# leotimus/recommender-tensorflow

Hardware: AMD Instinct MI355X
Metric: examples/sec DeepFM batch=65536 (full train step) (higher is better)
Workload: dtype f32 (MLP GEMM operands: fp16 hi+lo split, 3 products, fp32 accumulate)

## Files before the change

include/mi355x_rec.h:

```cpp
#ifndef MI355X_REC_H
#define MI355X_REC_H

#include <stddef.h>
#include <stdint.h>

#ifdef __cplusplus
extern "C" {
#endif

typedef void* mi_stream_t;

enum mi_status {
  MI_OK = 0,
  MI_ERR_INVALID = -1,
  MI_ERR_UNSUPPORTED = -2,
  MI_ERR_LAUNCH = -3,
  MI_ERR_WORKSPACE = -4
};

int32_t mi_abi_version(void);
const char* mi_last_error(void);
const char* mi_build_info(void);

typedef struct mi_step_state {
// ... 90 lines not shown
  MI_OPT_ADAGRAD = 1,
  MI_OPT_FTRL = 2,
  MI_OPT_RMSPROP = 3,
  MI_OPT_SGD = 4
};

typedef struct mi_opt_hparams {
  int32_t kind;
  float lr;
  float beta1, beta2, epsilon;
  float lr_t;
  float decay, momentum;
  float lr_power, l1, l2;
} mi_opt_hparams;

int32_t mi_axpy(float* y, const float* x, int64_t n, float alpha, mi_stream_t stream);

int32_t mi_dense_apply(float* param, float* slot0, float* slot1, const float* grad, int64_t n,
                       const mi_opt_hparams* hp, mi_stream_t stream);

int32_t mi_sparse_apply(float* table, float* t_slot0, float* t_slot1, float* lin_w, float* l_slot0,
                        float* l_slot1, int32_t* last_step, const int32_t* uniq_rows,
                        const int32_t* seg_start, const int32_t* sorted_entry,
                        const int32_t* num_uniq, int64_t n_max, const float* d_rows,
                        const float* d_lin, int32_t E, int32_t step, const mi_opt_hparams* hp,
                        int32_t lin_stride, int64_t table_stride, int64_t grad_stride, mi_stream_t stream);

int32_t mi_sparse_apply_fused(float* table, float* t_slot0, float* t_slot1, float* lin_w, float* l_slot0,
                              float* l_slot1, int32_t* last_step, const int32_t* uniq_rows,
                              const int32_t* seg_start, const int32_t* sorted_entry, const int32_t* num_uniq,
                              int64_t n_max, const float* d_concat, int64_t ld_dconcat, const float* sumv,
                              const float* d_logit_fm, const float* d_logit_lin, int32_t F, int32_t E,
                              int32_t step, const mi_opt_hparams* hp, int32_t lin_stride, int64_t table_stride, mi_stream_t stream);

enum mi_catchup_flags { MI_CATCHUP_DEFER_SLOTS = 1, MI_CATCHUP_BOUNDED = 2, MI_CATCHUP_KEEP_STAMPS = 4, MI_CATCHUP_LOCAL_ORDER = 8 };
int32_t mi_catchup_local_chunk_rows(void);
int32_t mi_catchup_bounded_runs(float beta1, float beta2, float epsilon);
int32_t mi_catchup_local_plan(int64_t n_max, int64_t num_uniq, int64_t* plan);
int32_t mi_catchup_gap_keys(const int32_t* uniq_rows, const int32_t* num_uniq, const int32_t* last_step, int64_t n_max,
                            int32_t step_to, int32_t* keys, int32_t lin_stride, mi_stream_t stream);

int32_t mi_catchup_rows_by_gap(const int32_t* uniq_rows, const int32_t* num_uniq, const int32_t* last_step, int64_t n_max,
                               int32_t step_to, int32_t lin_stride, int32_t* rows_out, void* workspace,
                               size_t workspace_bytes, mi_stream_t stream);


int32_t mi_selftest_sqrt(uint32_t first_bits, int64_t count, uint64_t* mismatches, mi_stream_t stream);

int32_t mi_selftest_div(float d, uint32_t first_bits, int64_t count, uint64_t* out, mi_stream_t stream);

int32_t mi_sparse_catchup(float* table, float* t_m, float* t_v, float* lin_w, float* l_m, float* l_v,
                          int32_t* last_step, const int32_t* uniq_rows, const int32_t* num_uniq,
                          int64_t n_max, int32_t E, int32_t step_to, const float* lr_table,
                          float beta1, float beta2, float epsilon, int32_t flags, int32_t lin_stride,
                          int64_t table_stride, mi_stream_t stream);


int32_t mi_set_gemm_mode(int32_t mode);
int32_t mi_get_gemm_mode(void);

#define MI_AMAX_SLOTS 64
typedef struct mi_gemm_amax {
  const float* a;
  const float* b;
  float* out;
} mi_gemm_amax_t;
// ... 238 lines not shown
```

recommender-tensorflow_amd/csrc/optim.hip:

```cpp
#include "common.h"
#include "optim_rules.h"
#include <algorithm>

namespace {

constexpr int kBlock = 256;

__global__ __launch_bounds__(kBlock) void dense_apply_k(float* __restrict__ w, float* __restrict__ s0,
                                                        float* __restrict__ s1,
                                                        const float* __restrict__ g, int64_t n,
                                                        Hp h, const mi_step_state_t* __restrict__ st) {
  if (st) h.lr_t = st->lr_t;
  const int64_t stride = static_cast<int64_t>(gridDim.x) * kBlock;
  for (int64_t i = static_cast<int64_t>(blockIdx.x) * kBlock + threadIdx.x; i < n; i += stride) {
    float wv = w[i], a = s0 ? s0[i] : 0.f, b = s1 ? s1[i] : 0.f;
    dense_rule(h, wv, a, b, g[i]);
    w[i] = wv;
    if (s0) s0[i] = a;
    if (s1) s1[i] = b;
  }
}

typedef float f32x4_t __attribute__((ext_vector_type(4)));
__device__ __forceinline__ float4 ld4_nt(const float* p) {
  const f32x4_t v = __builtin_nontemporal_load(reinterpret_cast<const f32x4_t*>(p));
  return make_float4(v[0], v[1], v[2], v[3]);
}
__device__ __forceinline__ void st4_nt(float* p, float4 v) {
  const f32x4_t x = {v.x, v.y, v.z, v.w};
  __builtin_nontemporal_store(x, reinterpret_cast<f32x4_t*>(p));
}

struct FusedGrad {
  const float* d_concat; int64_t ldd; const float* sumv; const float* dlf; const float* dll; int F;
  int64_t b0;
};

constexpr int kLongSeg = 48;
constexpr int kRun = 1;

struct ApplyArgs {
  float* table; float* t0; float* t1;
  float* lin_w; float* l0; float* l1;
  int32_t* last_step;
  const int32_t* uniq_rows; const int32_t* seg_start; const int32_t* sorted_entry; const int32_t* num_uniq;
  const float* d_rows; const float* d_lin;
  int E, step;
  float* out_rows; float* out_lin; int u_begin, u_count;
  int ls;
  const mi_step_state_t* st;
  int64_t ts;
  int64_t gs, gls, os, ols;
};

template <bool FUSED>
__device__ __forceinline__ void seg_accumulate(const ApplyArgs& a, const FusedGrad& fg, int k_beg, int k_end, int l,
                                               bool lane_on, const float4& w, float4& g, float& gl) {
  const int E = a.E;
  for (int k = k_beg; k < k_end; ++k) {
    const int64_t e = a.sorted_entry[k];
    if constexpr (FUSED) {
      const int64_t bg = e / fg.F;
      const int f = static_cast<int>(e - bg * fg.F);
      const int64_t b = bg - fg.b0;
      if (a.table && lane_on) {
        float4 v = make_float4(0.f, 0.f, 0.f, 0.f);
        if (fg.d_concat) v = ld4(fg.d_concat + b * fg.ldd + static_cast<int64_t>(f) * E + 4 * l);
        if (fg.dlf) {
          const float gf = fg.dlf[b];
          if (fg.sumv) {
            const float4 sv = ld4(fg.sumv + b * E + 4 * l);
            v.x += gf * (sv.x - w.x); v.y += gf * (sv.y - w.y);
            v.z += gf * (sv.z - w.z); v.w += gf * (sv.w - w.w);
          } else {
            v.x -= gf * w.x; v.y -= gf * w.y; v.z -= gf * w.z; v.w -= gf * w.w;
          }
        }
        g.x += v.x; g.y += v.y; g.z += v.z; g.w += v.w;
      }
      if (a.lin_w && l == 0) gl += fg.dll[b];
    } else {
      if (a.table && lane_on) {
        const float4 v = ld4(a.d_rows + e * a.gs + 4 * l);
        g.x += v.x; g.y += v.y; g.z += v.z; g.w += v.w;
      }
      if (a.lin_w && l == 0) gl += a.d_lin[e * a.gls];
// ... 38 lines not shown
    sparse_rule(h, w.z, s0.z, s1.z, g.z);
    sparse_rule(h, w.w, s0.w, s1.w, g.w);
    st4(a.table + o, w);
    if (a.t0) st4_nt(a.t0 + o, s0);
    if (a.t1) st4_nt(a.t1 + o, s1);
  }
  if (l == 0) {
    if (a.lin_w) {
      const int64_t o = r * a.ls;
      float lw = q.lw, s0 = q.ls0, s1 = q.ls1;
      for (int j = 0; j < missed; ++j) { s0 = s0 * h.beta1; s1 = s1 * h.beta2; }
      sparse_rule(h, lw, s0, s1, gl);
      a.lin_w[o] = lw;
      if (a.l0) a.l0[o] = s0;
      if (a.l1) a.l1[o] = s1;
    }
    if (a.last_step) a.last_step[r * a.ls] = a.step;
  }
}

__device__ __forceinline__ void store_row(const ApplyArgs& a, int64_t u, int l, bool lane_on, const float4& g, float gl) {
  if (a.out_rows && lane_on) st4(a.out_rows + u * a.os + 4 * l, g);
  if (a.out_lin && l == 0) a.out_lin[u * a.ols] = gl;
}

template <int LPR, bool FUSED, bool STORE = false>
__global__ __launch_bounds__(kBlock) void sparse_apply_k(ApplyArgs a, Hp h, const FusedGrad fg) {
  if (a.st) { a.step = a.st->step; h.lr_t = a.st->lr_t; }
  int64_t u = (static_cast<int64_t>(blockIdx.x) * kBlock + threadIdx.x) / LPR;
  const int l = threadIdx.x & (LPR - 1);
  if (u >= (STORE ? a.u_count : *a.num_uniq)) return;
  if (STORE) u += a.u_begin;
  const int s_beg = a.seg_start[u], s_end = a.seg_start[u + 1];
  if (s_end - s_beg > kLongSeg) return;
  const int64_t r = STORE ? u : static_cast<int64_t>(a.uniq_rows[u]);
  const bool lane_on = 4 * l < a.E;
  float4 g = make_float4(0.f, 0.f, 0.f, 0.f);
  float gl = 0.f;
  float4 w = make_float4(0.f, 0.f, 0.f, 0.f);
  if (a.table && lane_on) w = ld4(a.table + r * a.ts + 4 * l);
  RowState q;
  if constexpr (!STORE) q = load_row_state(a, h, r, l, lane_on);
  seg_accumulate<FUSED>(a, fg, s_beg, s_end, l, lane_on, w, g, gl);
  if constexpr (STORE) store_row(a, u, l, lane_on, g, gl);
  else apply_row(a, h, r, l, lane_on, w, g, gl, q);
}

template <int LPR, bool FUSED, bool STORE = false>
__global__ __launch_bounds__(kBlock) void sparse_apply_long_k(ApplyArgs a, Hp h, const FusedGrad fg) {
  if (a.st) { a.step = a.st->step; h.lr_t = a.st->lr_t; }
  constexpr int G = kBlock / LPR;
  __shared__ int list[kBlock];
  __shared__ int n_list;
  __shared__ float4 part[kBlock];
  __shared__ float part_l[G];
  const int U = STORE ? a.u_count : *a.num_uniq;
  const int ub = STORE ? a.u_begin : 0;
  const int t = threadIdx.x, l = t & (LPR - 1), grp = t / LPR;
  const bool lane_on = 4 * l < a.E;
  const int64_t per_round = static_cast<int64_t>(kBlock) * gridDim.x;
  {
    int any = 0;
    for (int64_t base = 0; base < U; base += per_round) {
      const int64_t u = base + (static_cast<int64_t>(t / kRun) * gridDim.x + blockIdx.x) * kRun + t % kRun;
      if (u < U) any |= (a.seg_start[ub + u + 1] - a.seg_start[ub + u] > kLongSeg) ? 1 : 0;
    }
    if (!__syncthreads_or(any)) return;
  }
  for (int64_t base = 0; base < U; base += per_round) {
    if (t == 0) n_list = 0;
    __syncthreads();
    const int64_t u = base + (static_cast<int64_t>(t / kRun) * gridDim.x + blockIdx.x) * kRun + t % kRun;
    if (u < U && a.seg_start[ub + u + 1] - a.seg_start[ub + u] > kLongSeg) list[atomicAdd(&n_list, 1)] = static_cast<int>(ub + u);
    __syncthreads();
    const int n = n_list;
    for (int j = 0; j < n; ++j) {
      const int uu = list[j];
      const int64_t r = STORE ? static_cast<int64_t>(uu) : static_cast<int64_t>(a.uniq_rows[uu]);
      const int s_beg = a.seg_start[uu], s_end = a.seg_start[uu + 1];
      const int per = (s_end - s_beg + G - 1) / G;
      const int k0 = min(s_end, s_beg + grp * per), k1 = min(s_end, k0 + per);
      float4 g = make_float4(0.f, 0.f, 0.f, 0.f);
      float gl = 0.f;
      float4 w = make_float4(0.f, 0.f, 0.f, 0.f);
      if (a.table && lane_on) w = ld4(a.table + r * a.ts + 4 * l);
      seg_accumulate<FUSED>(a, fg, k0, k1, l, lane_on, w, g, gl);
      part[t] = g;
      if (l == 0) part_l[grp] = gl;
      __syncthreads();
      if (grp == 0) {
        g = part[l];
        gl = part_l[0];
#pragma unroll 4
        for (int q = 1; q < G; ++q) {
          const float4 v = part[q * LPR + l];
          g.x += v.x; g.y += v.y; g.z += v.z; g.w += v.w;
          gl += part_l[q];
        }
        if constexpr (STORE) store_row(a, uu, l, lane_on, g, gl);
        else apply_row(a, h, r, l, lane_on, w, g, gl, load_row_state(a, h, r, l, lane_on));
      }
      __syncthreads();
    }
  }
}

__device__ __forceinline__ float sqrt_rn_fixup(float x) {
  float s = __builtin_amdgcn_sqrtf(x);
  const float sm = __uint_as_float(__float_as_uint(s) - 1u), sp = __uint_as_float(__float_as_uint(s) + 1u);
  const float rm = fmaf(-sm, s, x), rp = fmaf(-sp, s, x);
  s = (rm <= 0.f) ? sm : s;
  s = (rp > 0.f) ? sp : s;
  return s;
}
__device__ __forceinline__ float sqrt_rn_inrange(float x) {
  const float r = __builtin_amdgcn_rsqf(x);
  float s = x * r, h = 0.5f * r;
  const float e = fmaf(-h, s, 0.5f);
  h = fmaf(h, e, h);
  s = fmaf(s, e, s);
  const float d = fmaf(-s, s, x);
  return fmaf(d, h, s);
}
__device__ __forceinline__ float div_rn_inrange(float n, float d) {
  float r = __builtin_amdgcn_rcpf(d);
  const float e = fmaf(-d, r, 1.0f);
  r = fmaf(e, r, r);
  float q = n * r;
  const float e2 = fmaf(-d, q, n);
  q = fmaf(e2, r, q);
  const float e3 = fmaf(-d, q, n);
  return fmaf(e3, r, q);
}
__device__ __forceinline__ bool catchup_in_range(float m, float v) {
  const float am = fabsf(m);
  return (am == 0.f || (am >= 0x1p-50f && am <= 0x1p60f)) && v >= 0x1p-93f && v <= 0x1p20f;
}
// ... 454 lines not shown

#define MI_DISPATCH_LPR(lpr, CALL)                  \
  switch (lpr) {                                    \
    case 1: { constexpr int L = 1; CALL; } break;   \
    case 2: { constexpr int L = 2; CALL; } break;   \
    case 4: { constexpr int L = 4; CALL; } break;   \
    case 8: { constexpr int L = 8; CALL; } break;   \
    case 16: { constexpr int L = 16; CALL; } break; \
    case 32: { constexpr int L = 32; CALL; } break; \
    default: { constexpr int L = 64; CALL; } break; \
  }

static int32_t check_hp(const char* who, const mi_opt_hparams* hp) {
  if (!hp || hp->kind < MI_OPT_ADAM || hp->kind > MI_OPT_SGD) {
    mi::set_error("%s: bad optimizer kind", who);
    return MI_ERR_INVALID;
  }
  if (hp->kind == MI_OPT_FTRL && hp->lr_power != -0.5f) {
    mi::set_error("%s: Ftrl learning_rate_power %f unsupported (TF default -0.5 only)", who, hp->lr_power);
    return MI_ERR_UNSUPPORTED;
  }
  return MI_OK;
}

__global__ __launch_bounds__(kBlock) void axpy_k(float* __restrict__ y, const float* __restrict__ x, int64_t n, float alpha) {
  const int64_t i = static_cast<int64_t>(blockIdx.x) * kBlock + threadIdx.x;
  if (i < n) y[i] = y[i] + alpha * x[i];
}

unsigned long_grid(int64_t n_max) {
  return static_cast<unsigned>(std::min<int64_t>(1024, mi::ceil_div(n_max, kBlock)));
}

__global__ void step_advance_k(mi_step_state_t* __restrict__ st, const float* __restrict__ lr_table) {
  const int s = st->step + 1;
  st->step = s;
  st->lr_t = lr_table ? lr_table[s] : 0.f;
  st->seed_term = static_cast<uint64_t>(s) * 1000003ull;
}

extern "C" {

int32_t mi_step_advance(mi_step_state_t* device_state, const float* lr_table, mi_stream_t stream) {
  MI_REQUIRE(device_state, "step_advance: null state");
  step_advance_k<<<dim3(1), dim3(1), 0, mi::as_stream(stream)>>>(device_state, lr_table);
  MI_CHECK_LAUNCH("step_advance");
  return MI_OK;
}

int32_t mi_axpy(float* y, const float* x, int64_t n, float alpha, mi_stream_t stream) {
  MI_REQUIRE(n >= 0 && (n == 0 || (x && y)), "axpy: n=%lld", (long long)n);
  if (n == 0) return MI_OK;
  axpy_k<<<dim3((unsigned)mi::ceil_div(n, kBlock)), dim3(kBlock), 0, mi::as_stream(stream)>>>(y, x, n, alpha);
  MI_CHECK_LAUNCH("axpy");
  return MI_OK;
}


int32_t mi_dense_apply(float* param, float* slot0, float* slot1, const float* grad, int64_t n,
                       const mi_opt_hparams* hp, mi_stream_t stream) {
  if (int32_t rc = check_hp("dense_apply", hp)) return rc;
  MI_REQUIRE(n >= 0, "dense_apply: n=%lld", (long long)n);
  if (n == 0) return MI_OK;
  MI_REQUIRE(param && grad, "dense_apply: null buffer");
  MI_REQUIRE(hp->kind == MI_OPT_SGD || slot0, "dense_apply: optimizer needs slot0");
  MI_REQUIRE((hp->kind != MI_OPT_ADAM && hp->kind != MI_OPT_FTRL && hp->kind != MI_OPT_RMSPROP) || slot1,
             "dense_apply: optimizer needs slot1");
  int64_t nb = mi::ceil_div(n, kBlock);
  if (nb > 4096) nb = 4096;
  dense_apply_k<<<dim3((unsigned)nb), dim3(kBlock), 0, mi::as_stream(stream)>>>(param, slot0, slot1, grad, n, make_hp(hp), mi::step_state());
  MI_CHECK_LAUNCH("dense_apply");
  return MI_OK;
}

int32_t mi_sparse_apply(float* table, float* t_slot0, float* t_slot1, float* lin_w, float* l_slot0,
                        float* l_slot1, int32_t* last_step, const int32_t* uniq_rows,
                        const int32_t* seg_start, const int32_t* sorted_entry,
                        const int32_t* num_uniq, int64_t n_max, const float* d_rows,
                        const float* d_lin, int32_t E, int32_t step, const mi_opt_hparams* hp,
                        int32_t lin_stride, int64_t table_stride, int64_t grad_stride, mi_stream_t stream) {
  if (int32_t rc = check_hp("sparse_apply", hp)) return rc;
  MI_REQUIRE(grad_stride == 0 || (grad_stride >= (table ? E : 1) && (!table || (grad_stride & 3) == 0)),
             "sparse_apply: grad_stride=%lld (0 = d_rows E apart and d_lin 1 apart, else one record per entry)", (long long)grad_stride);
  if (!table) table_stride = 0;
  MI_REQUIRE(table_stride == 0 || (table_stride >= E && (table_stride & 3) == 0), "%s: table_stride=%lld (0 = E, else >= E and a multiple of 4)", "sparse_apply", (long long)table_stride);
  const int64_t ts = table_stride ? table_stride : E;

  MI_REQUIRE(lin_stride >= 1, "sparse_apply: lin_stride=%d", lin_stride);
  MI_REQUIRE(n_max >= 0, "sparse_apply: n_max=%lld", (long long)n_max);
  if (n_max == 0) return MI_OK;
  MI_REQUIRE(table || lin_w, "sparse_apply: nothing to update");
  MI_REQUIRE(uniq_rows && seg_start && sorted_entry && num_uniq, "sparse_apply: null index buffer");
  MI_REQUIRE(!table || (d_rows && E >= 4 && E <= 256 && (E & 3) == 0 && mi::aligned16(table) && mi::aligned16(d_rows)),
             "sparse_apply: table needs d_rows, E multiple of 4 in [4,256], 16-byte alignment");
  MI_REQUIRE(!lin_w || d_lin, "sparse_apply: lin_w needs d_lin");
  const bool need0 = hp->kind != MI_OPT_SGD;
  const bool need1 = hp->kind == MI_OPT_ADAM || hp->kind == MI_OPT_FTRL || hp->kind == MI_OPT_RMSPROP;
  MI_REQUIRE(!table || ((!need0 || t_slot0) && (!need1 || t_slot1)), "sparse_apply: table slots missing");
  MI_REQUIRE(!lin_w || ((!need0 || l_slot0) && (!need1 || l_slot1)), "sparse_apply: linear slots missing");
  const int lpr = table ? lanes_per_row(E) : 1;
  const int64_t blocks = mi::ceil_div(n_max * lpr, kBlock);
  MI_REQUIRE(blocks <= INT32_MAX, "sparse_apply: grid too large");
  const Hp h = make_hp(hp);
  ApplyArgs a{table, t_slot0, t_slot1, lin_w, l_slot0, l_slot1, last_step, uniq_rows, seg_start, sorted_entry,
              num_uniq, d_rows, d_lin, E, step};
  a.ls = lin_stride; a.ts = ts;
  a.gs = grad_stride ? grad_stride : E; a.gls = grad_stride ? grad_stride : 1;
  a.st = mi::step_state();
  MI_DISPATCH_LPR(lpr, (sparse_apply_k<L, false><<<dim3((unsigned)blocks), dim3(kBlock), 0, mi::as_stream(stream)>>>(
                           a, h, FusedGrad{})));
  MI_CHECK_LAUNCH("sparse_apply");
  if (n_max > kLongSeg) {
    MI_DISPATCH_LPR(lpr, (sparse_apply_long_k<L, false><<<dim3(long_grid(n_max)), dim3(kBlock), 0, mi::as_stream(stream)>>>(
                             a, h, FusedGrad{})));
    MI_CHECK_LAUNCH("sparse_apply(long segments)");
  }
  return MI_OK;
}

int32_t mi_sparse_apply_fused(float* table, float* t_slot0, float* t_slot1, float* lin_w, float* l_slot0,
                              float* l_slot1, int32_t* last_step, const int32_t* uniq_rows,
                              const int32_t* seg_start, const int32_t* sorted_entry, const int32_t* num_uniq,
                              int64_t n_max, const float* d_concat, int64_t ld_dconcat, const float* sumv,
                              const float* d_logit_fm, const float* d_logit_lin, int32_t F, int32_t E,
                              int32_t step, const mi_opt_hparams* hp, int32_t lin_stride, int64_t table_stride, mi_stream_t stream) {
  if (int32_t rc = check_hp("sparse_apply_fused", hp)) return rc;
  if (!table) table_stride = 0;
  MI_REQUIRE(table_stride == 0 || (table_stride >= E && (table_stride & 3) == 0), "%s: table_stride=%lld (0 = E, else >= E and a multiple of 4)", "sparse_apply_fused", (long long)table_stride);
  const int64_t ts = table_stride ? table_stride : E;

  MI_REQUIRE(lin_stride >= 1, "sparse_apply_fused: lin_stride=%d", lin_stride);
  MI_REQUIRE(n_max >= 0 && F > 0, "sparse_apply_fused: n_max=%lld F=%d", (long long)n_max, F);
  if (n_max == 0) return MI_OK;
  MI_REQUIRE(table || lin_w, "sparse_apply_fused: nothing to update");
  MI_REQUIRE(uniq_rows && seg_start && sorted_entry && num_uniq, "sparse_apply_fused: null index buffer");
  MI_REQUIRE(!table || (E >= 4 && E <= 256 && (E & 3) == 0 && mi::aligned16(table)),
             "sparse_apply_fused: E multiple of 4 in [4,256], 16-byte alignment");
  MI_REQUIRE(!table || d_concat || d_logit_fm, "sparse_apply_fused: table update needs d_concat and/or d_logit_fm");
  MI_REQUIRE(!d_concat || (ld_dconcat >= (int64_t)F * E && (ld_dconcat & 3) == 0 && mi::aligned16(d_concat)),
             "sparse_apply_fused: d_concat leading dimension / alignment");
  MI_REQUIRE(!d_logit_fm || (sumv ? mi::aligned16(sumv) : d_concat != nullptr),
             "sparse_apply_fused: FM gradient needs sumv, or a d_concat that already carries d_logit_fm * sumv");
  MI_REQUIRE(!lin_w || d_logit_lin, "sparse_apply_fused: lin_w needs d_logit_lin");
  const bool need0 = hp->kind != MI_OPT_SGD;
  const bool need1 = hp->kind == MI_OPT_ADAM || hp->kind == MI_OPT_FTRL || hp->kind == MI_OPT_RMSPROP;
  MI_REQUIRE(!table || ((!need0 || t_slot0) && (!need1 || t_slot1)), "sparse_apply_fused: table slots missing");
  MI_REQUIRE(!lin_w || ((!need0 || l_slot0) && (!need1 || l_slot1)), "sparse_apply_fused: linear slots missing");
  const int lpr = table ? lanes_per_row(E) : 1;
  const int64_t blocks = mi::ceil_div(n_max * lpr, kBlock);
  MI_REQUIRE(blocks <= INT32_MAX, "sparse_apply_fused: grid too large");
  const Hp h = make_hp(hp);
  const FusedGrad fg{d_concat, ld_dconcat, sumv, d_logit_fm, d_logit_lin, F, 0};
  ApplyArgs a{table, t_slot0, t_slot1, lin_w, l_slot0, l_slot1, last_step, uniq_rows, seg_start, sorted_entry,
              num_uniq, nullptr, nullptr, E, step};
  a.ls = lin_stride; a.ts = ts;
  a.st = mi::step_state();
  MI_DISPATCH_LPR(lpr, (sparse_apply_k<L, true><<<dim3((unsigned)blocks), dim3(kBlock), 0, mi::as_stream(stream)>>>(a, h, fg)));
  MI_CHECK_LAUNCH("sparse_apply_fused");
  if (n_max > kLongSeg) {
    MI_DISPATCH_LPR(lpr, (sparse_apply_long_k<L, true><<<dim3(long_grid(n_max)), dim3(kBlock), 0, mi::as_stream(stream)>>>(a, h, fg)));
    MI_CHECK_LAUNCH("sparse_apply_fused(long segments)");
  }
  return MI_OK;
}

int32_t mi_entry_grads_segsum(const float* rows, const int32_t* seg_start, const int32_t* sorted_entry, int64_t u_begin,
                              int64_t u_count, const float* d_concat, int64_t ld_dconcat, const float* sumv,
                              const float* d_logit_fm, const float* d_logit_lin, int64_t b0, int32_t F, int32_t E,
                              float* out_rows, float* out_lin, int64_t out_row0, int64_t rows_stride, int64_t out_stride,
                              mi_stream_t stream) {
  MI_REQUIRE(rows_stride == 0 || (rows_stride >= E && (rows_stride & 3) == 0), "entry_grads_segsum: rows_stride=%lld", (long long)rows_stride);
  MI_REQUIRE(out_stride == 0 || (out_stride >= (out_rows ? E : 1) && (!out_rows || (out_stride & 3) == 0)),
             "entry_grads_segsum: out_stride=%lld (0 = out_rows E apart and out_lin 1 apart, else one record per request)", (long long)out_stride);
  MI_REQUIRE(u_begin >= 0 && u_count >= 0 && u_begin + u_count <= INT32_MAX && F > 0 && b0 >= 0, "entry_grads_segsum: u_begin=%lld u_count=%lld",
             (long long)u_begin, (long long)u_count);
  MI_REQUIRE(out_row0 >= 0 && out_row0 <= u_begin, "entry_grads_segsum: out_row0=%lld must lie in [0, u_begin=%lld]", (long long)out_row0,
             (long long)u_begin);
  if (u_count == 0) return MI_OK;
  MI_REQUIRE(seg_start && sorted_entry && (out_rows || out_lin), "entry_grads_segsum: null buffer");
  MI_REQUIRE(!out_rows || (E >= 4 && E <= 256 && (E & 3) == 0 && mi::aligned16(out_rows) && (d_concat || d_logit_fm)),
             "entry_grads_segsum: row gradients need E multiple of 4 in [4,256] and d_concat and/or d_logit_fm");
  MI_REQUIRE(!d_concat || (ld_dconcat >= (int64_t)F * E && (ld_dconcat & 3) == 0 && mi::aligned16(d_concat)),
             "entry_grads_segsum: d_concat leading dimension / alignment");
  MI_REQUIRE(!d_logit_fm || (sumv && rows && mi::aligned16(sumv) && mi::aligned16(rows)), "entry_grads_segsum: the FM gradient needs sumv and the rows");
  MI_REQUIRE(!out_lin || d_logit_lin, "entry_grads_segsum: out_lin needs d_logit_lin");
  const int lpr = out_rows ? lanes_per_row(E) : 1;
  const int64_t blocks = mi::ceil_div(u_count * lpr, kBlock);
  MI_REQUIRE(blocks <= INT32_MAX, "entry_grads_segsum: grid too large");
  const FusedGrad fg{d_concat, ld_dconcat, sumv, d_logit_fm, d_logit_lin, F, b0};
  ApplyArgs a{};
  a.table = out_rows ? const_cast<float*>(rows) : nullptr;
  if (out_rows && !rows) a.table = out_rows;
  a.lin_w = out_lin;
  a.seg_start = seg_start; a.sorted_entry = sorted_entry;
  a.E = E;
  a.os = out_stride ? out_stride : E; a.ols = out_stride ? out_stride : 1;
  a.out_rows = out_rows ? reinterpret_cast<float*>(reinterpret_cast<uintptr_t>(out_rows) - static_cast<uintptr_t>(out_row0) * a.os * sizeof(float)) : nullptr;
  a.out_lin = out_lin ? reinterpret_cast<float*>(reinterpret_cast<uintptr_t>(out_lin) - static_cast<uintptr_t>(out_row0) * a.ols * sizeof(float)) : nullptr;
  a.u_begin = (int)u_begin; a.u_count = (int)u_count; a.ls = 1;
  a.ts = rows_stride ? rows_stride : E;
  const Hp h{};
  MI_DISPATCH_LPR(lpr, (sparse_apply_k<L, true, true><<<dim3((unsigned)blocks), dim3(kBlock), 0, mi::as_stream(stream)>>>(a, h, fg)));
  MI_CHECK_LAUNCH("entry_grads_segsum");
  if (u_count > 0) {
    MI_DISPATCH_LPR(lpr, (sparse_apply_long_k<L, true, true><<<dim3(long_grid(u_count)), dim3(kBlock), 0, mi::as_stream(stream)>>>(a, h, fg)));
    MI_CHECK_LAUNCH("entry_grads_segsum(long segments)");
  }
  return MI_OK;
}

int32_t mi_selftest_sqrt(uint32_t first_bits, int64_t count, uint64_t* mismatches, mi_stream_t stream) {
  MI_REQUIRE(count >= 0 && static_cast<uint64_t>(first_bits) + static_cast<uint64_t>(count) <= (1ull << 32), "selftest_sqrt: range leaves 32 bits");
  if (count == 0) return MI_OK;
  MI_REQUIRE(mismatches, "selftest_sqrt: null buffer");
  const int64_t blocks = mi::ceil_div(count, kBlock);
  MI_REQUIRE(blocks <= INT32_MAX, "selftest_sqrt: grid too large");
  selftest_sqrt_k<<<dim3((unsigned)blocks), dim3(kBlock), 0, mi::as_stream(stream)>>>(
      first_bits, count, reinterpret_cast<unsigned long long*>(mismatches));
  MI_CHECK_LAUNCH("selftest_sqrt");
  return MI_OK;
}

int32_t mi_catchup_gap_keys(const int32_t* uniq_rows, const int32_t* num_uniq, const int32_t* last_step, int64_t n_max,
                            int32_t step_to, int32_t* keys, int32_t lin_stride, mi_stream_t stream) {
  MI_REQUIRE(n_max >= 0 && step_to >= 0 && lin_stride >= 1, "catchup_gap_keys: n_max=%lld", (long long)n_max);
  if (n_max == 0) return MI_OK;
  MI_REQUIRE(uniq_rows && num_uniq && last_step && keys, "catchup_gap_keys: null buffer");
  gap_keys_k<<<dim3((unsigned)mi::ceil_div(n_max, kBlock)), dim3(kBlock), 0, mi::as_stream(stream)>>>(
      uniq_rows, num_uniq, last_step, n_max, step_to, keys, lin_stride, mi::step_state());
  MI_CHECK_LAUNCH("catchup_gap_keys");
  return MI_OK;
}

int32_t mi_catchup_local_chunk_rows(void) { return kLocalChunk; }
// ... 76 lines not shown
```

recommender-tensorflow_amd/mi355x_rec/_lib.py:

```python
import ctypes as C
import os

import torch

_HERE = os.path.dirname(os.path.abspath(__file__))
LIB_PATH = os.path.join(_HERE, "libmi355x_rec.so")

ABI_VERSION = 21


class MiError(RuntimeError):
    pass


class OptHparams(C.Structure):
    _fields_ = [("kind", C.c_int32), ("lr", C.c_float), ("beta1", C.c_float), ("beta2", C.c_float),
                ("epsilon", C.c_float), ("lr_t", C.c_float), ("decay", C.c_float),
                ("momentum", C.c_float), ("lr_power", C.c_float), ("l1", C.c_float),
                ("l2", C.c_float)]


AMAX_SLOTS = 64
MAX_WEIGHT_JOBS = 8

# ... 73 lines not shown
    "mi_step_advance": (_i32, [_p, _p, _p]),
    "mi_fingerprint64": (_u64, [_p, _sz]),
    "mi_crc32c": (_u32, [_p, _sz, _u32]),
    "mi_hash_bucket_i64": (_i32, [_p, _i64, _i64, _p]),
    "mi_hash_bucket_bytes": (_i32, [_p, _p, _i64, _i64, _p]),
    "mi_bucketize_f32": (_i32, [_p, _i64, _p, _i32, _p]),
    "mi_embed_fm_linear_fwd": (_i32, [_p, _p, _p, _p, _i64, _i32, _i32, _p, _i64, _p, _p, _p, _p, _i32, _i64, _p]),
    "mi_gather_rows": (_i32, [_p, _p, _p, _i64, _i32, _p, _p, _i32, _i64, _i64, _p]),
    "mi_numeric_embed_fwd": (_i32, [_p, _p, _p, _i64, _i32, _i32, _p, _i64, _i64, _p, _p, _p, _p]),
    "mi_numeric_raw_fwd": (_i32, [_p, _p, _i64, _i32, _p, _i64, _i64, _i32, _p, _p]),
    "mi_numeric_raw_bwd_workspace_bytes": (_sz, [_i64, _i32]),
    "mi_numeric_raw_bwd": (_i32, [_p, _p, _i64, _i32, _p, _p, _sz, _p]),
    "mi_embed_fm_linear_bwd": (_i32, [_p, _i64, _p, _i64, _p, _p, _p, _p, _p, _i64, _i32, _i32, _p, _p, _p]),
    "mi_entry_grads_segsum": (_i32, [_p, _p, _p, _i64, _i64, _p, _i64, _p, _p, _p, _i64, _i32, _i32, _p, _p, _i64, _i64, _i64, _p]),
    "mi_numeric_embed_bwd_workspace_bytes": (_sz, [_i64, _i32, _i32]),
    "mi_numeric_embed_bwd": (_i32, [_p, _p, _i64, _p, _i64, _i64, _p, _p, _p, _i64, _i32, _i32, _p,
                                    _p, _p, _sz, _p]),
    "mi_sort_unique_workspace_bytes": (_sz, [_i64]),
    "mi_sort_unique_fields_workspace_bytes": (_sz, [_i64, _i32]),
    "mi_sort_unique_fields": (_i32, [_p, _p, _i64, _i32, _i64, _p, _p, _p, _p, _p, _sz, _i32, _p]),
    "mi_sort_unique_rows": (_i32, [_p, _i64, _i64, _p, _p, _p, _p, _p, _sz, _p]),
    "mi_sort_unique_rows_slots": (_i32, [_p, _i64, _i64, _p, _p, _p, _p, _p, _p, _sz, _p]),
    "mi_global_rows": (_i32, [_p, _p, _i64, _i32, _p, _p]),
    "mi_shard_keys": (_i32, [_p, _i64, _i32, _i64, _i64, _i32, _p, _p]),
    "mi_route_requests": (_i32, [_p, _p, _i64, _i64, _i32, _p, _p, _p]),
    "mi_segment_slots": (_i32, [_p, _p, _p, _i64, _p, _p]),
    "mi_axpy": (_i32, [_p, _p, _i64, _f32, _p]),
    "mi_gather_u32": (_i32, [_p, _p, _i64, _p, _p]),
    "mi_dense_apply": (_i32, [_p, _p, _p, _p, _i64, C.POINTER(OptHparams), _p]),
    "mi_sparse_apply": (_i32, [_p, _p, _p, _p, _p, _p, _p, _p, _p, _p, _p, _i64, _p, _p, _i32, _i32,
                               C.POINTER(OptHparams), _i32, _i64, _i64, _p]),
    "mi_sparse_apply_fused": (_i32, [_p, _p, _p, _p, _p, _p, _p, _p, _p, _p, _p, _i64, _p, _i64, _p, _p, _p, _i32,
                                     _i32, _i32, C.POINTER(OptHparams), _i32, _i64, _p]),
    "mi_dense_fwd_gathered": (_i32, [_p, _p, _p, _i32, _i32, _p, _p, _p, _i64, _i64, _i32, _i32, _f32, _u64, _amax, _i64, _p]),
    "mi_dense_bwd_weight_gathered": (_i32, [_p, _p, _p, _i32, _i32, _p, _i64, _p, _p, _i64, _i32, _p, _sz, _amax, _i64, _p]),
    "mi_selftest_sqrt": (_i32, [_u32, _i64, _p, _p]),
    "mi_selftest_div": (_i32, [_f32, _u32, _i64, _p, _p]),
    "mi_catchup_gap_keys": (_i32, [_p, _p, _p, _i64, _i32, _p, _i32, _p]),
    "mi_catchup_rows_by_gap": (_i32, [_p, _p, _p, _i64, _i32, _i32, _p, _p, _sz, _p]),
    "mi_catchup_local_chunk_rows": (_i32, []),
    "mi_catchup_local_plan": (_i32, [_i64, _i64, _p]),
    "mi_catchup_bounded_runs": (_i32, [_f32, _f32, _f32]),
    "mi_sparse_catchup": (_i32, [_p, _p, _p, _p, _p, _p, _p, _p, _p, _i64, _i32, _i32, _p, _f32, _f32,
                                 _f32, _i32, _i32, _i64, _p]),
    "mi_set_gemm_mode": (_i32, [_i32]),
    "mi_absmax": (_i32, [_p, _i64, _p, _p]),
    "mi_get_gemm_mode": (_i32, []),
    "mi_dense_fwd": (_i32, [_p, _i64, _p, _p, _p, _i64, _i64, _i32, _i32, _i32, _f32, _u64, _amax, _p]),
    "mi_dense_bwd_data": (_i32, [_p, _i64, _p, _p, _i64, _p, _i64, _i64, _i32, _i32, _f32, _i32, _amax, _p]),
    "mi_dense_bwd_weight_workspace_bytes": (_sz, [_i64, _i32, _i32]),
    "mi_dense_bwd_data_vec_planes": (_i32, [_p, _i64, _p, _p, _i64, _f32, _p, _i64, _pl, _i64, _i32, _p, _p, _i64, _p]),
    "mi_dense_bwd_weight_planes_workspace_bytes": (_sz, [_i64, _i32, _i32]),
    "mi_dense_bwd_weight_planes": (_i32, [_p, _p, _p, _p, _i64, _i32, _i32, _p, _sz, _p, _p]),
    "mi_dense_bwd_weight": (_i32, [_p, _i64, _p, _i64, _p, _p, _i64, _i32, _i32, _p, _sz, _amax, _p]),
    "mi_dense_bwd_weight_planes_batch_workspace_bytes": (_sz, [_p, _i32, _i64]),
    "mi_dense_bwd_weight_planes_batch": (_i32, [_p, _i32, _i64, _p, _sz, _p]),
    "mi_planes_bytes": (_sz, [_i64, _i32]),
    "mi_split_rows": (_i32, [_p, _i64, _i64, _i32, _i32, _pl, _p, _p]),
    "mi_split_weights": (_i32, [_p, _p, _i32, _p, _p]),
    "mi_merge_rows": (_i32, [_pl, _i64, _i32, _p, _i64, _p]),
    "mi_dense_fwd_planes": (_i32, [_pl, _pl, _p, _p, _i64, _pl, _i64, _i32, _i32, _i32, _f32, _u64, _p, _p, _i64, _p]),
    "mi_dense_bwd_data_planes": (_i32, [_pl, _pl, _pl, _p, _i64, _pl, _i64, _i32, _i32, _f32, _p, _p, _i64, _p]),
    "mi_embed_fm_planes_fwd": (_i32, [_p, _p, _p, _i64, _i32, _i32, _p, _p, _pl, _p, _p, _i32, _i32, _i64, _p]),
    "mi_logits_head_fused_workspace_bytes": (_sz, [_i64, _i32]),
    "mi_logits_head_fused": (_i32, [_p, _i64, _p, _p, _p, _p, _p, _p, _i64, _i32, _f32, _p, _i64, _f32, _p, _p, _p, _p, _p, _p, _p, _pl,
                                    _p, _i64, _p, _p, _sz, _p]),
# ... 92 lines not shown
```

recommender-tensorflow_amd/mi355x_rec/engine.py:

```python
import ctypes as C
import json
import os
import math

import numpy as np
import torch

from . import _lib
from ._lib import OptHparams, check, ptr

OPT_KINDS = {"Adam": 0, "Adagrad": 1, "Ftrl": 2, "RMSProp": 3, "SGD": 4}


def _align(n, a=16):
    return (n + a - 1) // a * a


def predict_buffers(B, device):
    cls = torch.empty(B, 1, dtype=torch.int64, device=device)
    return {"logits": torch.empty(B, 1, dtype=torch.float32, device=device),
            "logistic": torch.empty(B, 1, dtype=torch.float32, device=device),
            "probabilities": torch.empty(B, 2, dtype=torch.float32, device=device), "class_ids": cls, "classes": cls}


def check_members(who, engines, most, limit):
    engines = list(engines)
    if len(engines) < 1:
        raise ValueError("%s: no members" % who)
    if len(engines) > most:
        raise ValueError("%s: %d members (at most %d in one launch)" % (who, len(engines), most))
    lead = engines[0]
    for i, e in enumerate(engines):
        if e.device != lead.device:
            raise ValueError("%s: member %d is on %s, member 0 on %s" % (who, i, e.device, lead.device))
        if list(e.vocab_sizes) != list(lead.vocab_sizes) or e.n_numeric != lead.n_numeric:
            raise ValueError("%s: member %d has columns (%s buckets, %d numeric), member 0 (%s, %d)" % (
                who, i, list(e.vocab_sizes), e.n_numeric, list(lead.vocab_sizes), lead.n_numeric))
        why = limit(e)
        if why is not None:
            raise ValueError("%s: member %d: the model has %s" % (who, i, why))
    return engines


class HipKernels:

    supports_planes = True

    def __init__(self):
        self.lib = _lib.load()
        self.timers = None
        self.timer_only = None

    def query(self, name, *args):
        return getattr(self.lib, name)(*args)

    def tagged(self, name, tag):
        key = name + tag
        if key not in self.__dict__:
            self.__dict__[key] = self._bind(name, key)
        return self.__dict__[key]

    def __getattr__(self, name):
        if not name.startswith("mi_"):
            raise AttributeError(name)
        call = self.__dict__[name] = self._bind(name, name)
        return call

    def _bind(self, name, key):
        fn = getattr(self.lib, name)

        def call(*args):
            a = [ptr(x) if isinstance(x, torch.Tensor) else (C.byref(x) if isinstance(x, C.Structure) else x)
                 for x in args]
            a.append(_lib.cur_stream())
# ... 1121 lines not shown
            else:
                V = self._seg(self.dense, self.num_emb_off, (self.n_numeric, E))[jj].contiguous()
                k.mi_numeric_embed_fwd(x, V, wn, n, nx, E, concat, concat.shape[1], Fx * E, sumv, fm, lin)
        a = None
        if self.use_dnn:
            H1 = self.layers[0][3]
            rows = [f * E + j for f in cat for j in range(E)] if self.use_emb else []
            if raw:
                rows += [self.D_emb + j for j in num]
            else:
                rows += [self.F * E + j * E + e for j in num for e in range(E)]
            a = torch.empty(n, H1, **f32)
            b0 = self.bias(0) if candidate else torch.zeros(H1, **f32)
            if rows:
                W = torch.zeros(D, H1, **f32)
                W[:len(rows)] = self.kernel(0)[torch.tensor(rows, dtype=torch.int64, device=dev)]
                k.mi_dense_fwd(concat, concat.shape[1], W, b0, a, H1, n, H1, D, 0, 1.0, 0, None)
            else:
                a.copy_(b0.expand(n, H1))
        w = None
        if lin is not None or fm is not None:
            w = torch.empty(n, **f32)
            lb = self.dense[self.lin_bias_off:] if (candidate and self.use_linear) else None
            hws = self._bytes("topk_head_ws", k.query("mi_head_workspace_bytes", n))
            k.mi_sigmoid_ce_head(lin, lb, fm, None, None, n, 1.0, w, None, None, None, hws, hws.numel())
        elif candidate and self.use_linear:
            w = self.dense[self.lin_bias_off:self.lin_bias_off + 1].expand(n).contiguous()
        return a, sumv, w

    GAP_SORT_MIN = 16384
    TOP_FUSED_MIN_BATCH = 4096
    GRAPH_SHAPES_MAX = 4
    LOCAL_CATCHUP = True

    def _new_side_stream(self, priority=0):
        n = self.__dict__.setdefault("_n_side", {})
        k = n[priority] = n.get(priority, -1) + 1
        return _tested_side_stream(self.device, priority, k)

    def _catchup(self, uniq, num_uniq, n_max, defer=False, by_gap=None):
        t_adam = self.opt.name == "Adam" and self.table is not None
        l_adam = (self.lin_opt or self.opt).name == "Adam" and self.lin_w is not None
        if not (t_adam or l_adam) or n_max == 0:
            return
        defer = bool(defer and uniq is not None and self.lin_opt is None)
        for sc in (self.sched, self.lin_sched):
            if sc is not None:
                sc.lr_t(self.step)
        flags = (1 if defer else 0) | (2 if self.catchup == "bounded" else 0)
        t_sched = self.sched if t_adam else None
        l_sched = (self.lin_sched if self.lin_opt is not None else (self.lin_sched or self.sched)) if l_adam else None
        if self._local_catchup(defer, n_max):
            s = t_sched.spec
            self.k.mi_sparse_catchup(self.table, self.t_s0, self.t_s1, self.lin_w, self.l_s0, self.l_s1, self.last_step, uniq,
                                     num_uniq, n_max, self.E, self.step, t_sched.table, s.beta1, s.beta2, s.epsilon,
                                     flags | 8, self.ls, self.ts)
            return
        if uniq is not None and n_max >= self.GAP_SORT_MIN:
            uniq = by_gap if by_gap is not None else self._rows_by_gap(uniq, num_uniq, n_max, self.step)
        side = None
        if t_sched is not None and l_sched is not None and t_sched is not l_sched:
            assert not defer
            parts = [(None, l_sched, 4), (t_sched, None, 0)]
        elif (defer and t_sched is not None and l_sched is not None and self.shard is None and self.device.type == "cuda"
              and self._wide_on_side_stream(n_max // max(self.F, 1))):
            parts = [(None, l_sched, 0), (t_sched, None, 0)]
# ... 245 lines not shown
                                                   self._planes("dy%dp" % (i - 1), B, fan), B, fan, self._av("dy%d" % (i - 1)),
                                                   mb, 0 if mb is None else mb.shape[1])
                else:
                    k.mi_dense_bwd_data(dy, lddy, self.kernel(i), x if i else None, ldx, dx, fan, B, h, fan,
                                        keep if i else 1.0, self.act, None if self.planes else ga_d)
                    if self.planes and i == nh and i > 0:
                        k.mi_split_rows(dx, fan, B, fan, 0, self._planes("dy%dp" % (i - 1), B, fan), self._av("dy%d" % (i - 1)))
                if data_first:
                    on_d_concat(dx)
                    weight_gradient()
                dy, lddy = dx, fan
            d_concat = dy
            for lo in range(0, len(batch or ()), _lib.MAX_WEIGHT_JOBS):
                part = batch[lo:lo + _lib.MAX_WEIGHT_JOBS]
                arr = (_lib.WgradJob * len(part))()
                for q, (i, fan, h, ga_w) in enumerate(part):
                    arr[q].X, arr[q].dY = self._pl["x%dp" % i].struct, self._pl["dy%dp" % i].struct
                    arr[q].dW, arr[q].db = ptr(self.kernel(i, self.d_grad)), ptr(self.bias(i, self.d_grad))
                    arr[q].N, arr[q].K, arr[q].amax = h, fan, ga_w
                bws = self._bytes("wgrad_batch_ws", k.query("mi_dense_bwd_weight_planes_batch_workspace_bytes", arr, len(part), B))
                k.mi_dense_bwd_weight_planes_batch(arr, len(part), B, bws, bws.numel())
        if self.n_numeric and self.raw_numeric:
            if self.use_linear:
                ws = self._bytes("num_ws", k.query("mi_numeric_raw_bwd_workspace_bytes", B, self.n_numeric))
                k.mi_numeric_raw_bwd(c["x_num"], dlogit, B, self.n_numeric, self.d_grad[self.lin_num_off:], ws, ws.numel())
        elif self.n_numeric:
            ws = self._bytes("num_ws", k.query("mi_numeric_embed_bwd_workspace_bytes", B, self.n_numeric, self.E))
            k.mi_numeric_embed_bwd(c["x_num"], d_concat, self.D, c["concat"], self.D, self.F * self.E, c["sumv"],
                                   dlogit if self.use_mf else None, dlogit if self.use_linear else None, B,
                                   self.n_numeric, self.E, self.d_grad[self.num_emb_off:],
                                   self.d_grad[self.lin_num_off:] if self.use_linear else None, ws, ws.numel())
        return d_concat

    def _apply(self, uniq, seg, sorted_entry, num_uniq, n_max, d_rows, d_lin, fused=None):
        k = self.k
        step = self.step + 1
        lr_t = self.sched.lr_t(step) if self.sched else 0.0
        hp = self.opt.hparams(lr_t)
        lin_lr_t = self.lin_sched.lr_t(step) if self.lin_sched else 0.0
        if self._frozen is not None:
            self.d_grad.index_fill_(0, self._frozen, 0.0)
        if self.lin_opt is None:
            if self.P:
                k.mi_dense_apply(self.dense, self.d_s0, self.d_s1, self.d_grad, self.P, hp)
            sparse_hp = [(True, True, hp)]
        else:
            lhp = self.lin_opt.hparams(lin_lr_t)
            if self.wide_off:
                k.mi_dense_apply(self.dense, self.d_s0, self.d_s1, self.d_grad, self.wide_off, hp)
            o = self.wide_off
            sl = lambda t: t[o:] if t is not None else None
            k.mi_dense_apply(self.dense[o:], sl(self.dl_s0), sl(self.dl_s1), self.d_grad[o:], self.P - o, lhp)
            sparse_hp = [(True, False, hp), (False, True, lhp)]
        if n_max > 0:
            for do_table, do_lin, h in sparse_hp:
                tb = self.table if (do_table and self.use_emb) else None
                lw = self.lin_w if (do_lin and self.use_linear) else None
                if tb is None and lw is None:
                    continue
                slots = (tb, self.t_s0 if tb is not None else None, self.t_s1 if tb is not None else None,
                         lw, self.l_s0 if lw is not None else None, self.l_s1 if lw is not None else None)
                if fused is not None:
                    d_concat, sumv, dlogit = fused
                    k.mi_sparse_apply_fused(*slots, self.last_step, uniq, seg, sorted_entry, num_uniq, n_max,
                                            d_concat if tb is not None else None, self.D,
                                            sumv if (tb is not None and self.use_mf) else None,
                                            dlogit if (tb is not None and self.use_mf) else None,
                                            dlogit if lw is not None else None, self.F, self.E, step, h, self.ls, self.ts)
                else:
                    k.mi_sparse_apply(*slots, self.last_step, uniq, seg, sorted_entry, num_uniq, n_max,
                                      d_rows if tb is not None else None, d_lin if lw is not None else None, self.E,
                                      step, h, self.ls, self.ts, 0)
        self.step = step

    def graph_ok(self):
        return (self.shard is None and self.device.type == "cuda" and
                not (self.sched is not None and self.lin_sched is not None and self.sched is not self.lin_sched))

    def graph_train_step(self, ids, labels, x_num=None):
        if self.shard is not None or self.device.type != "cuda":
            raise NotImplementedError("graph_train_step: single-GPU models")
        if not self.graph_ok():
            raise NotImplementedError("graph_train_step: the device-resident step state carries ONE lr_t (two different Adams)")
        self._prep(ids, labels, x_num)
        graphs = self.__dict__.setdefault("_graphs", {})
        shape = tuple(ids.shape)
        g = self._graph = graphs.get(shape)
# ... 303 lines not shown
```

Baseline: 23.93 million.

## Record long-segment rows in a device hot list to skip rescan in long kernel

The short-segment sparse apply kernel now appends the indices of rows whose segments exceed the long threshold to a device scratch list via an atomic counter. The follow-up long-segment kernel reads this list and processes only those rows, instead of rescanning every unique row's segment bounds. The last block to finish resets the counters. This adds a global scratch buffer registered from Python, atomics, and cross-launch state that must stay consistent, for example under graph capture or when the list overflows.

Result: no change. 23.90 million (-0.1%).

```diff
diff --git a/include/mi355x_rec.h b/include/mi355x_rec.h
--- a/include/mi355x_rec.h
+++ b/include/mi355x_rec.h
@@ -146,6 +146,9 @@
                               int64_t n_max, const float* d_concat, int64_t ld_dconcat, const float* sumv,
                               const float* d_logit_fm, const float* d_logit_lin, int32_t F, int32_t E,
                               int32_t step, const mi_opt_hparams* hp, int32_t lin_stride, int64_t table_stride, mi_stream_t stream);
+
+size_t mi_apply_scratch_bytes(int64_t n_max);
+int32_t mi_set_apply_scratch(int32_t* device_buf, size_t bytes);
 
 enum mi_catchup_flags { MI_CATCHUP_DEFER_SLOTS = 1, MI_CATCHUP_BOUNDED = 2, MI_CATCHUP_KEEP_STAMPS = 4, MI_CATCHUP_LOCAL_ORDER = 8 };
 int32_t mi_catchup_local_chunk_rows(void);
diff --git a/recommender-tensorflow_amd/csrc/optim.hip b/recommender-tensorflow_amd/csrc/optim.hip
--- a/recommender-tensorflow_amd/csrc/optim.hip
+++ b/recommender-tensorflow_amd/csrc/optim.hip
@@ -51,7 +51,9 @@
   const mi_step_state_t* st;
   int64_t ts;
   int64_t gs, gls, os, ols;
+  int32_t* hot; int hot_cap;
 };
+constexpr int kHotHdr = 4;
 
 template <bool FUSED>
 __device__ __forceinline__ void seg_accumulate(const ApplyArgs& a, const FusedGrad& fg, int k_beg, int k_end, int l,
@@ -156,7 +158,13 @@
   if (u >= (STORE ? a.u_count : *a.num_uniq)) return;
   if (STORE) u += a.u_begin;
   const int s_beg = a.seg_start[u], s_end = a.seg_start[u + 1];
-  if (s_end - s_beg > kLongSeg) return;
+  if (s_end - s_beg > kLongSeg) {
+    if (a.hot && l == 0) {
+      const int p = atomicAdd(&a.hot[0], 1);
+      if (p < a.hot_cap) a.hot[kHotHdr + p] = static_cast<int>(u);
+    }
+    return;
+  }
   const int64_t r = STORE ? u : static_cast<int64_t>(a.uniq_rows[u]);
   const bool lane_on = 4 * l < a.E;
   float4 g = make_float4(0.f, 0.f, 0.f, 0.f);
@@ -170,6 +178,48 @@
   else apply_row(a, h, r, l, lane_on, w, g, gl, q);
 }
 
+template <int LPR, bool FUSED, bool STORE>
+__device__ __forceinline__ void apply_long_row(const ApplyArgs& a, const Hp& h, const FusedGrad& fg, int uu, float4* part,
+                                               float* part_l) {
+  constexpr int G = kBlock / LPR;
+  const int t = threadIdx.x, l = t & (LPR - 1), grp = t / LPR;
+  const bool lane_on = 4 * l < a.E;
+  const int64_t r = STORE ? static_cast<int64_t>(uu) : static_cast<int64_t>(a.uniq_rows[uu]);
+  const int s_beg = a.seg_start[uu], s_end = a.seg_start[uu + 1];
+  const int per = (s_end - s_beg + G - 1) / G;
+  const int k0 = min(s_end, s_beg + grp * per), k1 = min(s_end, k0 + per);
+  float4 g = make_float4(0.f, 0.f, 0.f, 0.f);
+  float gl = 0.f;
+  float4 w = make_float4(0.f, 0.f, 0.f, 0.f);
+  if (a.table && lane_on) w = ld4(a.table + r * a.ts + 4 * l);
+  seg_accumulate<FUSED>(a, fg, k0, k1, l, lane_on, w, g, gl);
+  part[t] = g;
+  if (l == 0) part_l[grp] = gl;
+  __syncthreads();
+  if (grp == 0) {
+    g = part[l];
+    gl = part_l[0];
+#pragma unroll 4
+    for (int q = 1; q < G; ++q) {
+      const float4 v = part[q * LPR + l];
+      g.x += v.x; g.y += v.y; g.z += v.z; g.w += v.w;
+      gl += part_l[q];
+    }
+    if constexpr (STORE) store_row(a, uu, l, lane_on, g, gl);
+    else apply_row(a, h, r, l, lane_on, w, g, gl, load_row_state(a, h, r, l, lane_on));
+  }
+  __syncthreads();
+}
+
+__device__ __forceinline__ void hot_list_leave(int32_t* hot) {
+  if (threadIdx.x == 0) {
+    if (atomicAdd(&hot[1], 1) == static_cast<int>(gridDim.x) - 1) {
+      __atomic_store_n(&hot[0], 0, __ATOMIC_RELAXED);
+      __atomic_store_n(&hot[1], 0, __ATOMIC_RELAXED);
+    }
+  }
+}
+
 template <int LPR, bool FUSED, bool STORE = false>
 __global__ __launch_bounds__(kBlock) void sparse_apply_long_k(ApplyArgs a, Hp h, const FusedGrad fg) {
   if (a.st) { a.step = a.st->step; h.lr_t = a.st->lr_t; }
@@ -178,10 +228,21 @@
   __shared__ int n_list;
   __shared__ float4 part[kBlock];
   __shared__ float part_l[G];
+  const int t = threadIdx.x;
+  if (a.hot) {
+    if (t == 0) n_list = __atomic_load_n(&a.hot[0], __ATOMIC_RELAXED);
+    __syncthreads();
+    const int n = n_list;
+    if (n == 0) return;
+    if (n <= a.hot_cap) {
+      for (int j = blockIdx.x; j < n; j += gridDim.x) apply_long_row<LPR, FUSED, STORE>(a, h, fg, a.hot[kHotHdr + j], part, part_l);
+      hot_list_leave(a.hot);
+      return;
+    }
+    __syncthreads();
+  }
   const int U = STORE ? a.u_count : *a.num_uniq;
   const int ub = STORE ? a.u_begin : 0;
-  const int t = threadIdx.x, l = t & (LPR - 1), grp = t / LPR;
-  const bool lane_on = 4 * l < a.E;
   const int64_t per_round = static_cast<int64_t>(kBlock) * gridDim.x;
   {
     int any = 0;
@@ -189,7 +250,10 @@
       const int64_t u = base + (static_cast<int64_t>(t / kRun) * gridDim.x + blockIdx.x) * kRun + t % kRun;
       if (u < U) any |= (a.seg_start[ub + u + 1] - a.seg_start[ub + u] > kLongSeg) ? 1 : 0;
     }
-    if (!__syncthreads_or(any)) return;
+    if (!__syncthreads_or(any)) {
+      if (a.hot) hot_list_leave(a.hot);
+      return;
+    }
   }
   for (int64_t base = 0; base < U; base += per_round) {
     if (t == 0) n_list = 0;
@@ -198,35 +262,9 @@
     if (u < U && a.seg_start[ub + u + 1] - a.seg_start[ub + u] > kLongSeg) list[atomicAdd(&n_list, 1)] = static_cast<int>(ub + u);
     __syncthreads();
     const int n = n_list;
-    for (int j = 0; j < n; ++j) {
-      const int uu = list[j];
-      const int64_t r = STORE ? static_cast<int64_t>(uu) : static_cast<int64_t>(a.uniq_rows[uu]);
-      const int s_beg = a.seg_start[uu], s_end = a.seg_start[uu + 1];
-      const int per = (s_end - s_beg + G - 1) / G;
-      const int k0 = min(s_end, s_beg + grp * per), k1 = min(s_end, k0 + per);
-      float4 g = make_float4(0.f, 0.f, 0.f, 0.f);
-      float gl = 0.f;
-      float4 w = make_float4(0.f, 0.f, 0.f, 0.f);
-      if (a.table && lane_on) w = ld4(a.table + r * a.ts + 4 * l);
-      seg_accumulate<FUSED>(a, fg, k0, k1, l, lane_on, w, g, gl);
-      part[t] = g;
-      if (l == 0) part_l[grp] = gl;
-      __syncthreads();
-      if (grp == 0) {
-        g = part[l];
-        gl = part_l[0];
-#pragma unroll 4
-        for (int q = 1; q < G; ++q) {
-          const float4 v = part[q * LPR + l];
-          g.x += v.x; g.y += v.y; g.z += v.z; g.w += v.w;
-          gl += part_l[q];
-        }
-        if constexpr (STORE) store_row(a, uu, l, lane_on, g, gl);
-        else apply_row(a, h, r, l, lane_on, w, g, gl, load_row_state(a, h, r, l, lane_on));
-      }
-      __syncthreads();
-    }
-  }
+    for (int j = 0; j < n; ++j) apply_long_row<LPR, FUSED, STORE>(a, h, fg, list[j], part, part_l);
+  }
+  if (a.hot) hot_list_leave(a.hot);
 }
 
 __device__ __forceinline__ float sqrt_rn_fixup(float x) {
@@ -747,6 +785,17 @@
   return static_cast<unsigned>(std::min<int64_t>(1024, mi::ceil_div(n_max, kBlock)));
 }
 
+struct HotScratch { int32_t* buf; int64_t cap; int device; };
+HotScratch g_hot{nullptr, 0, -1};
+void use_hot_list(ApplyArgs& a, int64_t rows_max) {
+  a.hot = nullptr; a.hot_cap = 0;
+  if (!g_hot.buf || g_hot.cap < rows_max) return;
+  int dev = -1;
+  if (hipGetDevice(&dev) != hipSuccess || dev != g_hot.device) return;
+  a.hot = g_hot.buf;
+  a.hot_cap = static_cast<int>(std::min<int64_t>(g_hot.cap, INT32_MAX));
+}
+
 __global__ void step_advance_k(mi_step_state_t* __restrict__ st, const float* __restrict__ lr_table) {
   const int s = st->step + 1;
   st->step = s;
@@ -761,6 +810,24 @@
   step_advance_k<<<dim3(1), dim3(1), 0, mi::as_stream(stream)>>>(device_state, lr_table);
   MI_CHECK_LAUNCH("step_advance");
   return MI_OK;
+}
+
+int32_t mi_set_apply_scratch(int32_t* device_buf, size_t bytes) {
+  if (!device_buf) { g_hot = HotScratch{nullptr, 0, -1}; return MI_OK; }
+  MI_REQUIRE((reinterpret_cast<uintptr_t>(device_buf) & 3u) == 0 && bytes >= (kHotHdr + 1) * sizeof(int32_t),
+             "set_apply_scratch: %zu bytes (a 4-byte aligned buffer of at least %zu)", bytes, (kHotHdr + 1) * sizeof(int32_t));
+  hipPointerAttribute_t at{};
+  if (hipPointerGetAttributes(&at, device_buf) != hipSuccess || at.type != hipMemoryTypeDevice) {
+    (void)hipGetLastError();
+    mi::set_error("set_apply_scratch: not device memory");
+    return MI_ERR_INVALID;
+  }
+  g_hot = HotScratch{device_buf, static_cast<int64_t>(bytes / sizeof(int32_t)) - kHotHdr, at.device};
+  return MI_OK;
+}
+
+size_t mi_apply_scratch_bytes(int64_t n_max) {
+  return (kHotHdr + static_cast<size_t>(std::max<int64_t>(1, n_max / (kLongSeg + 1)))) * sizeof(int32_t);
 }
 
 int32_t mi_axpy(float* y, const float* x, int64_t n, float alpha, mi_stream_t stream) {
@@ -822,6 +889,7 @@
   a.ls = lin_stride; a.ts = ts;
   a.gs = grad_stride ? grad_stride : E; a.gls = grad_stride ? grad_stride : 1;
   a.st = mi::step_state();
+  use_hot_list(a, n_max / (kLongSeg + 1));
   MI_DISPATCH_LPR(lpr, (sparse_apply_k<L, false><<<dim3((unsigned)blocks), dim3(kBlock), 0, mi::as_stream(stream)>>>(
                            a, h, FusedGrad{})));
   MI_CHECK_LAUNCH("sparse_apply");
@@ -870,6 +938,7 @@
               num_uniq, nullptr, nullptr, E, step};
   a.ls = lin_stride; a.ts = ts;
   a.st = mi::step_state();
+  use_hot_list(a, n_max / (kLongSeg + 1));
   MI_DISPATCH_LPR(lpr, (sparse_apply_k<L, true><<<dim3((unsigned)blocks), dim3(kBlock), 0, mi::as_stream(stream)>>>(a, h, fg)));
   MI_CHECK_LAUNCH("sparse_apply_fused");
   if (n_max > kLongSeg) {
@@ -915,6 +984,7 @@
   a.u_begin = (int)u_begin; a.u_count = (int)u_count; a.ls = 1;
   a.ts = rows_stride ? rows_stride : E;
   const Hp h{};
+  use_hot_list(a, u_count);
   MI_DISPATCH_LPR(lpr, (sparse_apply_k<L, true, true><<<dim3((unsigned)blocks), dim3(kBlock), 0, mi::as_stream(stream)>>>(a, h, fg)));
   MI_CHECK_LAUNCH("entry_grads_segsum");
   if (u_count > 0) {
diff --git a/recommender-tensorflow_amd/mi355x_rec/_lib.py b/recommender-tensorflow_amd/mi355x_rec/_lib.py
--- a/recommender-tensorflow_amd/mi355x_rec/_lib.py
+++ b/recommender-tensorflow_amd/mi355x_rec/_lib.py
@@ -129,6 +129,8 @@
                                C.POINTER(OptHparams), _i32, _i64, _i64, _p]),
     "mi_sparse_apply_fused": (_i32, [_p, _p, _p, _p, _p, _p, _p, _p, _p, _p, _p, _i64, _p, _i64, _p, _p, _p, _i32,
                                      _i32, _i32, C.POINTER(OptHparams), _i32, _i64, _p]),
+    "mi_apply_scratch_bytes": (_sz, [_i64]),
+    "mi_set_apply_scratch": (_i32, [_p, _sz]),
     "mi_dense_fwd_gathered": (_i32, [_p, _p, _p, _i32, _i32, _p, _p, _p, _i64, _i64, _i32, _i32, _f32, _u64, _amax, _i64, _p]),
     "mi_dense_bwd_weight_gathered": (_i32, [_p, _p, _p, _i32, _i32, _p, _i64, _p, _p, _i64, _i32, _p, _sz, _amax, _i64, _p]),
     "mi_selftest_sqrt": (_i32, [_u32, _i64, _p, _p]),
diff --git a/recommender-tensorflow_amd/mi355x_rec/engine.py b/recommender-tensorflow_amd/mi355x_rec/engine.py
--- a/recommender-tensorflow_amd/mi355x_rec/engine.py
+++ b/recommender-tensorflow_amd/mi355x_rec/engine.py
@@ -40,6 +40,9 @@
         if why is not None:
             raise ValueError("%s: member %d: the model has %s" % (who, i, why))
     return engines
+
+
+_HOT_ROWS = {"reg": None, "bufs": {}, "outgrown": []}
 
 
 class HipKernels:
@@ -1227,6 +1230,7 @@
     TOP_FUSED_MIN_BATCH = 4096
     GRAPH_SHAPES_MAX = 4
     LOCAL_CATCHUP = True
+    HOT_ROW_LIST = True
 
     def _new_side_stream(self, priority=0):
         n = self.__dict__.setdefault("_n_side", {})
@@ -1538,6 +1542,30 @@
                                    self.d_grad[self.lin_num_off:] if self.use_linear else None, ws, ws.numel())
         return d_concat
 
+    def _hot_row_list(self, n_max):
+        k = self.k
+        if self.device.type != "cuda" or not hasattr(k, "mi_set_apply_scratch"):
+            return
+        st = _HOT_ROWS
+        if not self.HOT_ROW_LIST:
+            if st["reg"] is not None:
+                k.query("mi_set_apply_scratch", None, 0)
+                st["reg"] = None
+            return
+        need = k.query("mi_apply_scratch_bytes", n_max)
+        buf = st["bufs"].get(self.device)
+        if (buf is None or buf.numel() * 4 < need) and not getattr(self, "_capturing", False):
+            if buf is not None:
+                st["outgrown"].append(buf)
+            buf = st["bufs"][self.device] = torch.zeros((need + 3) // 4, dtype=torch.int32, device=self.device)
+            torch.cuda.current_stream().synchronize()
+        if buf is None:
+            return
+        reg = (buf.data_ptr(), buf.numel() * 4)
+        if st["reg"] != reg:
+            _lib.check(k.query("mi_set_apply_scratch", reg[0], reg[1]), "mi_set_apply_scratch")
+            st["reg"] = reg
+
     def _apply(self, uniq, seg, sorted_entry, num_uniq, n_max, d_rows, d_lin, fused=None):
         k = self.k
         step = self.step + 1
@@ -1559,6 +1587,7 @@
             k.mi_dense_apply(self.dense[o:], sl(self.dl_s0), sl(self.dl_s1), self.d_grad[o:], self.P - o, lhp)
             sparse_hp = [(True, False, hp), (False, True, lhp)]
         if n_max > 0:
+            self._hot_row_list(n_max)
             for do_table, do_lin, h in sparse_hp:
                 tb = self.table if (do_table and self.use_emb) else None
                 lw = self.lin_w if (do_lin and self.use_linear) else None
```
